# rrwick/Porechop

Measured on NVIDIA H100. Metric: reads/sec, higher is better.
Workload: dtype int16 (s16x2 DPX)

## Files before the change

porechop_b200/csrc/dp_core.cuh:

```cuda
#pragma once
#include <stdint.h>

#if defined(__CUDACC__)
#define PB_HD __host__ __device__ __forceinline__
#else
#define PB_HD inline
#endif

namespace pb {

#if !defined(__CUDA_ARCH__) && defined(PB_CHECK_RANGES)
void pb_range_violation();
#endif

constexpr int PB_BIAS = 24576;
constexpr int PB_NEG16 = -14000;
constexpr int PB_I16_LIMIT = 4000;
constexpr int PB_LINEAR_EXT = 4096;
constexpr int PB_CODE_SHIFT = 12;
constexpr int PB_MAX_SUBW = 4096;
constexpr uint8_t PB_PAD_H = 0x50;
constexpr uint8_t PB_PAD_V = 0x60;

constexpr int PB_REC = 9;
// ... 243 lines not shown
PB_HD uint32_t profile_from(uint32_t v2, uint32_t sf2, uint32_t bcode, const Scoring &sc) {
    const uint32_t e = (bcode & 7u) << 4;
    const uint32_t h2 = (e << 8) | (e << 24);
    return addmax2(xnor2(h2, v2), sc.subA2, sf2);
}
PB_HD uint32_t profile_plain(uint32_t sub2) { return (sub2 & 0x8000u) ? sub2 - 0x10000u : sub2; }
#define PB_PROF_ENCODE(x) profile_plain(x)
PB_HD uint32_t profile_word(int q, uint32_t bcode, const Scoring &sc, const uint8_t *adA, int mA, int padA, const uint8_t *adB,
                            int mB, int padB) {
    uint32_t v2, sf2;
    profile_row(q, sc, adA, mA, padA, adB, mB, padB, v2, sf2);
    return profile_from(v2, sf2, bcode, sc);
}

template <int R> struct TraceWords { static constexpr int value = (R <= 4) ? 1 : 2; };
template <int R> PB_HD int trace_word(int h, int r) { (void)r; return (R <= 4) ? 0 : h; }
template <int R> PB_HD int trace_shift(int h, int r) { return (R <= 4) ? (4 * r + 16 * h) : 4 * r; }

PB_HD int corr_flags(int x, int vs, int hs, int goEff) {
    const int sb = x - goEff;
    return (vs == sb ? 1 : 0) | (hs == sb ? 2 : 0);
}
struct FinalCol { int mask; int i0[2]; };
template <int R>
PB_HD void final_col_row(Lane<R> &L, const FinalCol &fc, int r, uint32_t x, uint32_t vs, uint32_t hs, const Scoring &sc) {
#pragma unroll
    for (int h = 0; h < 2; ++h) {
        const int i = fc.i0[h] + r;
        if (((fc.mask >> h) & 1) && i >= 1) {
            const int c = half16(x, h);
            if (c > L.fcBest[h]) {
                L.fcBest[h] = c; L.fcI[h] = i;
                L.fcCorr[h] = corr_flags(c, half16(vs, h), half16(hs, h), sc.goEff);
            }
        }
    }
}

#define PB_EXT(x) add2((x), sc.ge2)
template <int R, bool TRACE, bool KEEPV = false, bool PROF = false, bool FCOL = false>
PB_HD void lane_step(Lane<R> &L, uint32_t recvX, uint32_t recvV, uint32_t h2, const Scoring &sc, uint32_t *tw,
                     uint32_t *vr = nullptr, const uint32_t *subs = nullptr, const FinalCol *fc = nullptr) {
    uint32_t diagX = L.prevRecvX, upX = recvX, upV = recvV;
    uint32_t accLo = 0u, accHi = 0u;
#pragma unroll
    for (int r = 0; r < R; ++r) {
        const uint32_t sub = PROF ? subs[r] : addmax2(xnor2(h2, L.v2[r]), sc.subA2, L.sf2[r]);
        const uint32_t d = PROF ? diagX + sub : add2(diagX, sub);
#if !defined(__CUDA_ARCH__) && defined(PB_CHECK_RANGES)
        if (PROF && d != add2(diagX, (sub & 0x8000u) ? sub + 0x10000u : sub)) pb_range_violation();
#endif
        uint32_t hs, vs, s;
        if (TRACE) {
            const uint32_t bl = 1u << trace_shift<R>(0, r);
            const uint32_t bh = 1u << trace_shift<R>(1, r);
            const int alu_sites = (r & 1) ? (PB_FLAG_ALU_B) : (PB_FLAG_ALU_A);
            hs = max2acc((alu_sites & 1) != 0, PB_EXT(L.Hs[r]), L.X[r], accLo, bl << 3, accHi, bh << 3);
            vs = max2acc((alu_sites & 2) != 0, PB_EXT(upV), upX, accLo, bl << 2, accHi, bh << 2);
            const uint32_t gmx = max2acc((alu_sites & 4) != 0, vs, hs, accLo, bl << 1, accHi, bh << 1);
            s = max2acc((alu_sites & 8) != 0, d, gmx, accLo, bl, accHi, bh);
        } else {
            hs = addmax2(L.Hs[r], sc.ge2, L.X[r]);
            vs = addmax2(upV, sc.ge2, upX);
            s = max3(d, vs, hs);
        }
        diagX = L.X[r];
        const uint32_t xn = subm2(s, sc.goMag2);
        L.X[r] = xn; L.Hs[r] = hs;
        if (KEEPV) vr[r] = vs;
        if (FCOL) final_col_row<R>(L, *fc, r, xn, vs, hs, sc);
        upX = xn; upV = vs;
    }
    if (TRACE) {
        if (TraceWords<R>::value == 1) tw[0] = accLo + accHi; else { tw[0] = accLo; tw[1] = accHi; }
    }
    L.prevRecvX = recvX;
    L.botX = upX; L.botV = upV;
}

template <int R>
PB_HD void lane_track_lastrow(Lane<R> &L, int j, const Scoring &sc) {
    bool plo, phi;
    const uint32_t nb = max2p(L.lrBest2, L.botX, plo, phi);
    (void)sc;
    if (!(plo && phi)) {
        L.lrBest2 = nb;
        if (!plo) { L.lrJ[0] = j; L.lrV2 = (L.lrV2 & 0xFFFF0000u) | (L.botV & 0xFFFFu); L.lrH2 = (L.lrH2 & 0xFFFF0000u) | (L.Hs[R - 1] & 0xFFFFu); }
        if (!phi) { L.lrJ[1] = j; L.lrV2 = (L.lrV2 & 0xFFFFu) | (L.botV & 0xFFFF0000u); L.lrH2 = (L.lrH2 & 0xFFFFu) | (L.Hs[R - 1] & 0xFFFF0000u); }
    }
}

template <int R, bool FCOL = true>
PB_HD void lane_track_general(Lane<R> &L, int g, int j, const HalfGeom &A, const HalfGeom &B, const uint32_t *vr,
                              const Scoring &sc) {
#pragma unroll
    for (int h = 0; h < 2; ++h) {
        const HalfGeom &H = h ? B : A;
        if (j < H.n) {
            const int c = half16(L.botX, h);
            if (c > half16(L.lrBest2, h)) {
                const uint32_t keep = h ? 0xFFFFu : 0xFFFF0000u;
                L.lrBest2 = (L.lrBest2 & keep) | (L.botX & ~keep);
                L.lrV2 = (L.lrV2 & keep) | (L.botV & ~keep);
                L.lrH2 = (L.lrH2 & keep) | (L.Hs[R - 1] & ~keep);
                L.lrJ[h] = j;
            }
        } else if (FCOL && j == H.n) {
#pragma unroll
            for (int r = 0; r < R; ++r) {
                const int i = g * R + r + 1 - H.pad;
                if (i >= 1) {
                    const int c = half16(L.X[r], h);
                    if (c > L.fcBest[h]) {
                        L.fcBest[h] = c; L.fcI[h] = i;
                        L.fcCorr[h] = corr_flags(c, half16(vr[r], h), half16(L.Hs[r], h), sc.goEff);
                    }
                }
            }
        }
    }
}

struct ScoutCand { int fcBest, fcI, fcCorr, lrBest, lrJ, lrCorr; };
template <int R>
PB_HD ScoutCand make_cand(const Lane<R> &L, int h, const Scoring &sc) {
    ScoutCand c;
    c.fcBest = L.fcBest[h] < 0 ? -0x40000000 : L.fcBest[h] - PB_BIAS - sc.goEff;
    c.fcI = L.fcI[h]; c.fcCorr = L.fcCorr[h];
    c.lrBest = half16(L.lrBest2, h) - PB_BIAS - sc.goEff; c.lrJ = L.lrJ[h];
    c.lrCorr = L.lrJ[h] > 0 ? corr_flags(half16(L.lrBest2, h), half16(L.lrV2, h), half16(L.lrH2, h), sc.goEff) : 0;
    return c;
}
PB_HD EndCell scout_combine(const ScoutCand *c, int G, const HalfGeom &H) {
    EndCell e;
    if (H.n <= 0 || H.m <= 0) { e.j = 0; e.i = 0; e.score = PB_SCORE_EMPTY; e.corr = 0; return e; }
    const ScoutCand &lr = c[G - 1];
    int best = lr.lrBest, bj = lr.lrJ, bi = H.m, corr = lr.lrCorr;
    for (int g = 0; g < G; ++g) {
        if (c[g].fcBest > best) { best = c[g].fcBest; bj = H.n; bi = c[g].fcI; corr = c[g].fcCorr; }
    }
    e.j = bj; e.i = bi; e.score = best; e.corr = corr;
    return e;
}

template <class NibFn, class EqFn>
struct RandomCursor {
    NibFn nib; EqFn eqf; int j, i;
    PB_HD RandomCursor(NibFn n, EqFn e, int j0, int i0) : nib(n), eqf(e), j(j0), i(i0) {}
    PB_HD uint32_t flags() { return nib(j, i); }
    PB_HD bool eq() { return eqf(j, i); }
    PB_HD void move(bool consR, bool consA) { j -= consR ? 1 : 0; i -= consA ? 1 : 0; }
};

template <class Cursor>
PB_HD int traceback_stats_cur(Cursor &cur, const EndCell &end, bool linear, int col0, int n_total, int m, int32_t *rec) {
    if (end.score == PB_SCORE_EMPTY) {
        rec[0] = -1; rec[1] = 0; rec[2] = -1; rec[3] = 0; rec[4] = PB_SCORE_EMPTY;
        rec[5] = 0; rec[6] = 0; rec[7] = 0; rec[8] = 0;
        return 0;
    }
    int j = end.j, i = end.i;
    int L = 0, matches = 0;
    int pv = 0, ph = 0, tv = 0, th = 0;
    int dPV = 0, dPH = 0, dTV = 0, dTH = 0;
    int dir = 0;
    uint32_t b = 0;
    if (j > 0 && i > 0) {
        b = cur.flags();
        dir = (b & 1u) ? 0 : ((b & 2u) ? 1 : 2);
        if (!linear) {
            if (end.corr & 1) dir = 1; else if (end.corr & 2) dir = 2;
        }
    }
    while (j > 0 && i > 0) {
        const bool isD = dir == 0, isV = dir == 1, isH = dir == 2;
        const bool consR = !isV, consA = !isH;
        if (isD && cur.eq()) ++matches;
        const bool inPV = pv == L, inPH = ph == L;
        if (inPV) { if (isV) ++pv; else dPV = isD ? 1 : 0; }
        if (inPH) { if (isH) ++ph; else dPH = isD ? 1 : 0; }
        if (isV) ++tv; else { tv = 0; dTV = isD ? 1 : 0; }
        if (isH) ++th; else { th = 0; dTH = isD ? 1 : 0; }
        const bool ext = !linear && (isV ? ((b & 4u) && i != 1) : (isH && (b & 8u) && j != 1));
        ++L;
        if (consR) --j;
        if (consA) --i;
        cur.move(consR, consA);
        if (j > 0 && i > 0) {
            b = cur.flags();
            if (!ext) dir = (b & 1u) ? 0 : ((b & 2u) ? 1 : 2);
        }
    }
    const bool haveR = pv < L, haveA = ph < L;
    const int lastR_k = pv, lastR_i = end.i - pv, lastR_uA = dPV;
    const int lastA_k = ph, lastA_j = end.j - ph, lastA_uR = dPH;
    const int firstR_k = L - 1 - tv, firstR_i = i + tv + dTV, firstR_uA = dTV;
    const int firstA_k = L - 1 - th, firstA_j = j + th + dTH, firstA_uR = dTH;
    int status = (j == 0 && i > 0 && col0 > 0) ? 1 : 0;

    const int a = col0 + j, bb = i;
    const int jend = col0 + end.j;
    const int c = n_total - jend, e = m - end.i;
    const int Ltot = a + bb + L + c + e;
#define PB_COL(k) (a + bb + (L - 1 - (k)))
    int r0, AB_r0, a0, RB_a0;
    if (a > 0) { r0 = 0; AB_r0 = 0; }
    else if (haveR) { r0 = PB_COL(firstR_k); AB_r0 = firstR_i - firstR_uA; }
    else { r0 = bb + L; AB_r0 = end.i; }
    if (bb > 0) { a0 = 0; RB_a0 = 0; }
    else if (haveA) { a0 = PB_COL(firstA_k); RB_a0 = col0 + firstA_j - firstA_uR; }
    else { a0 = a + L + c; RB_a0 = n_total; }
    int rs, as;
    int start;
    if (r0 >= a0) { start = r0; rs = 0; as = AB_r0; } else { start = a0; as = 0; rs = RB_a0; }
    int r1, AB_r1, a1, RB_a1;
    if (c > 0) { r1 = Ltot - 1; AB_r1 = m; }
    else if (haveR) { r1 = PB_COL(lastR_k); AB_r1 = lastR_i - lastR_uA; }
    else { r1 = a - 1; AB_r1 = 0; }
    if (e > 0) { a1 = Ltot - 1; RB_a1 = n_total; }
    else if (haveA) { a1 = PB_COL(lastA_k); RB_a1 = col0 + lastA_j - lastA_uR; }
    else { a1 = a + bb - 1; RB_a1 = 0; }
#undef PB_COL
    int re, ae, endc;
    if (r1 <= a1) { endc = r1; re = n_total - 1; ae = AB_r1; } else { endc = a1; ae = m - 1; re = RB_a1; }
    rec[0] = rs; rec[1] = re; rec[2] = as; rec[3] = ae; rec[4] = end.score;
    rec[5] = matches; rec[6] = endc - start + 1; rec[7] = matches; rec[8] = a1 - a0 + 1;
    return status;
}

template <class NibFn, class EqFn>
PB_HD int traceback_stats(NibFn nib, EqFn eq, const EndCell &end, bool linear, int col0, int n_total, int m,
                          int32_t *rec) {
    RandomCursor<NibFn, EqFn> cur(nib, eq, end.j, end.i);
    return traceback_stats_cur(cur, end, linear, col0, n_total, m, rec);
}

PB_HD int32_t end_trim_candidate(const int32_t *r, int is_start, int32_t end_size, int32_t extra_trim, int32_t min_trim,
                                 const int32_t *cmin, int32_t cmin_len, int *overflow) {
    const bool failed = r[0] == -1 && r[4] == PB_SCORE_EMPTY;
    if (failed) return 0;
    const int32_t l = r[6], c = r[5];
    if (l < 0 || l >= cmin_len) { *overflow = 1; return 0; }
    if (c < cmin[l]) return 0;
    const int32_t rs = r[0], re = r[1] + 1;
    if (re - rs < min_trim) return 0;
    if (is_start) return (re == end_size) ? 0 : re + extra_trim;
    return (rs == 0) ? 0 : (end_size - rs) + extra_trim;
}
PB_HD bool middle_hit(const int32_t *r, const int32_t *cmin, int32_t cmin_len, int *overflow) {
    const int32_t l = r[8], c = r[7];
    if (l < 0 || l >= cmin_len) { *overflow = 1; return false; }
    return l > 0 && c >= cmin[l];
}
PB_HD uint32_t score_pair(const int32_t *r, int *overflow) {
    if (r[0] == -1 && r[4] == PB_SCORE_EMPTY) return 1u << 16;
    if ((uint32_t)r[7] > 0xFFFFu || (uint32_t)r[8] > 0xFFFFu) { *overflow = 1; return 0u; }
    return (uint32_t)r[7] | ((uint32_t)r[8] << 16);
}

}
```

porechop_b200/csrc/kernels.cuh:

```cuda
#pragma once
#include <cuda_runtime.h>
#include <stdint.h>
#include <string.h>
#include "dp_core.cuh"

namespace pb {

constexpr int PB_WARPS_PER_BLOCK = 4;
#ifndef PB_TRACE_MIN_BLOCKS
#define PB_TRACE_MIN_BLOCKS 6
#endif
#ifndef PB_TRACE_MIN_BLOCKS_WIDE
#define PB_TRACE_MIN_BLOCKS_WIDE 5
#endif
constexpr int PB_SCRATCH_WORDS = 32 * 2 * 6;
constexpr int PB_TCHUNK = 4;

__device__ __forceinline__ uint32_t encode_word(uint32_t w) {
    return encode_byte(w & 0xFFu) | (encode_byte((w >> 8) & 0xFFu) << 8) | (encode_byte((w >> 16) & 0xFFu) << 16) |
           (encode_byte(w >> 24) << 24);
}
__global__ void encode_kernel(const uint8_t *__restrict__ in, uint8_t *__restrict__ out, int64_t n) {
    int64_t i = ((int64_t)blockIdx.x * blockDim.x + threadIdx.x) * 16;
    const int64_t stride = (int64_t)gridDim.x * blockDim.x * 16;
    for (; i < n; i += stride) {
        if (i + 16 <= n && ((((uintptr_t)in) | ((uintptr_t)out)) & 15) == 0) {
            uint4 v = *reinterpret_cast<const uint4 *>(in + i);
            v.x = encode_word(v.x); v.y = encode_word(v.y); v.z = encode_word(v.z); v.w = encode_word(v.w);
            *reinterpret_cast<uint4 *>(out + i) = v;
        } else {
            for (int64_t k = i; k < n && k < i + 16; ++k) out[k] = (uint8_t)encode_byte(in[k]);
        }
    }
}

__global__ void unpack_kernel(const uint8_t *__restrict__ in, uint8_t *__restrict__ out, int64_t n) {
    int64_t i = ((int64_t)blockIdx.x * blockDim.x + threadIdx.x) * 16;
    const int64_t stride = (int64_t)gridDim.x * blockDim.x * 16;
    for (; i < n; i += stride) {
        if (i + 16 <= n && ((((uintptr_t)in) & 7) | (((uintptr_t)out) & 15)) == 0) {
            const uint2 p = *reinterpret_cast<const uint2 *>(in + (i >> 1));
            uint4 v;
            unpack_nibbles8(p.x, v.x, v.y);
            unpack_nibbles8(p.y, v.z, v.w);
            *reinterpret_cast<uint4 *>(out + i) = v;
        } else {
            for (int64_t k = i; k < n && k < i + 16; ++k) out[k] = (uint8_t)unpack_nibble1(in[k >> 1], (int)(k & 1));
        }
    }
}

__global__ void max_len_kernel(const int64_t *__restrict__ off, int64_t n, unsigned long long *out) {
    int64_t i = (int64_t)blockIdx.x * blockDim.x + threadIdx.x;
    unsigned long long v = 0;
    for (; i < n; i += (int64_t)gridDim.x * blockDim.x) {
        unsigned long long l = (unsigned long long)(off[i + 1] - off[i]);
        v = l > v ? l : v;
    }
    for (int o = 16; o > 0; o >>= 1) { unsigned long long w = __shfl_xor_sync(0xffffffffu, v, o); v = w > v ? w : v; }
    if ((threadIdx.x & 31) == 0 && v) atomicMax(out, v);
}

constexpr int PB_ORDER_BINS = 2048;
__device__ __forceinline__ int order_bin(int64_t len, int64_t max_len) {
    int64_t b = (len * (PB_ORDER_BINS - 1)) / (max_len > 0 ? max_len : 1);
    if (b > PB_ORDER_BINS - 1) b = PB_ORDER_BINS - 1;
    return (PB_ORDER_BINS - 1) - (int)b;
}
__global__ void order_hist_kernel(const int64_t *__restrict__ off, int64_t n, int64_t max_len, unsigned *__restrict__ bins) {
    int64_t i = (int64_t)blockIdx.x * blockDim.x + threadIdx.x;
    if (i < n) atomicAdd(&bins[order_bin(off[i + 1] - off[i], max_len)], 1u);
}
__global__ void order_scan_kernel(unsigned *bins) {
    __shared__ unsigned sh[PB_ORDER_BINS];
    for (int i = threadIdx.x; i < PB_ORDER_BINS; i += blockDim.x) sh[i] = bins[i];
    __syncthreads();
    if (threadIdx.x == 0) {
        unsigned run = 0;
        for (int i = 0; i < PB_ORDER_BINS; ++i) { unsigned v = sh[i]; sh[i] = run; run += v; }
    }
    __syncthreads();
    for (int i = threadIdx.x; i < PB_ORDER_BINS; i += blockDim.x) bins[i] = sh[i];
}
__global__ void order_scatter_kernel(const int64_t *__restrict__ off, int64_t n, int64_t max_len, unsigned *__restrict__ bins,
                                     int32_t *__restrict__ order) {
    int64_t i = (int64_t)blockIdx.x * blockDim.x + threadIdx.x;
    if (i < n) {
        unsigned pos = atomicAdd(&bins[order_bin(off[i + 1] - off[i], max_len)], 1u);
        order[pos] = (int32_t)i;
    }
}

struct TaskSrc {
    const Task *tasks;
    int64_t n_tasks;
    const int32_t *cls_ad;
    int32_t n_cls_ad;
    int32_t n_adapters;
    int64_t n_seqs;
    const int64_t *seq_off;
    const int32_t *ad_off;
    const int32_t *seq_order;
};

__device__ __forceinline__ Task cross_task(const TaskSrc &ts, int64_t k) {
    const int n_full = ts.n_cls_ad / 2;
    const int64_t paired = (int64_t)n_full * 2 * ts.n_seqs;
    int64_t s; int a;
    if (k < paired) {
        int64_t q, rem;
        if (paired <= 0xFFFFFFFFll) {
            const uint32_t d = (uint32_t)(2 * ts.n_seqs), q32 = (uint32_t)k / d;
            q = q32; rem = (uint32_t)k - q32 * d;
        } else {
            q = k / (2 * ts.n_seqs); rem = k - q * (2 * ts.n_seqs);
        }
        s = rem >> 1; a = __ldg(ts.cls_ad + 2 * q + (rem & 1));
    } else {
        s = k - paired; a = __ldg(ts.cls_ad + ts.n_cls_ad - 1);
    }
    if (ts.seq_order) s = __ldg(ts.seq_order + s);
    Task t;
    const int64_t o0 = __ldg(ts.seq_off + s), o1 = __ldg(ts.seq_off + s + 1);
    const int32_t a0 = __ldg(ts.ad_off + a), a1 = __ldg(ts.ad_off + a + 1);
    t.seq_off = o0;
    t.n = (int32_t)(o1 - o0);
    t.m = a1 - a0;
    t.ad_off = a0;
    t.out_idx = (int32_t)(s * ts.n_adapters + a);
    t.flags = 0; t.end_j = 0; t.end_i = 0; t.end_corr = 0; t.end_score = 0;
    t.col0 = 0; t.n_total = t.n; t.pad0 = t.pad1 = t.pad2 = 0;
    return t;
}
__global__ void build_tasks_pairs_kernel(Task *__restrict__ tasks, int64_t n_tasks, const int32_t *__restrict__ order,
                                         const int32_t *__restrict__ pair_seq, const int32_t *__restrict__ pair_ad,
                                         const int64_t *__restrict__ seq_off, const int32_t *__restrict__ ad_off) {
    int64_t k = (int64_t)blockIdx.x * blockDim.x + threadIdx.x;
    if (k >= n_tasks) return;
    int32_t p = order[k];
    int64_t s = pair_seq[p]; int a = pair_ad[p];
    Task t;
    t.seq_off = seq_off[s];
    t.n = (int32_t)(seq_off[s + 1] - seq_off[s]);
    t.m = ad_off[a + 1] - ad_off[a];
    t.ad_off = ad_off[a];
    t.out_idx = p;
    t.flags = 0; t.end_j = 0; t.end_i = 0; t.end_corr = 0; t.end_score = 0;
    t.col0 = 0; t.n_total = t.n; t.pad0 = t.pad1 = t.pad2 = 0;
    tasks[k] = t;
}

__device__ __forceinline__ Task get_task(const TaskSrc &ts, int64_t idx) {
    Task t;
    if (idx < ts.n_tasks) {
        if (ts.tasks == nullptr) return cross_task(ts, idx);
        const int4 *p = reinterpret_cast<const int4 *>(ts.tasks + idx);
        int4 *q = reinterpret_cast<int4 *>(&t);
        q[0] = __ldcs(p); q[1] = __ldcs(p + 1); q[2] = __ldcs(p + 2); q[3] = __ldcs(p + 3);
    } else {
        t.seq_off = 0; t.n = 0; t.m = 0; t.ad_off = 0; t.out_idx = -1; t.flags = 0; t.end_j = 0; t.end_i = 0;
        t.end_corr = 0; t.end_score = 0; t.col0 = 0; t.n_total = 0; t.pad0 = t.pad1 = t.pad2 = 0;
    }
    return t;
}

__global__ void window_tasks_kernel(const TaskSrc ts, const EndCell *__restrict__ ends, Task *__restrict__ out,
                                    int wnum, int wden, int tight, unsigned long long *__restrict__ window_cells) {
    const int64_t n_tasks = ts.n_tasks;
    int64_t k = (int64_t)blockIdx.x * blockDim.x + threadIdx.x;
    unsigned long long cells = 0;
    if (k < n_tasks) {
        Task t = get_task(ts, k);
        EndCell e = ends[k];
        if (t.n > 0 && t.m > 0) {
            const int64_t W = window_cols(t.m, e.i, e.score, wnum, wden, tight != 0);
            int64_t c0 = (int64_t)e.j - W;
            if (c0 < 0) c0 = 0;
            t.col0 = (int32_t)c0;
            t.seq_off += c0;
            t.n = e.j - (int32_t)c0;
            t.flags = TASK_END_GIVEN | (c0 > 0 ? TASK_LEFT_INF : 0);
            t.end_j = t.n; t.end_i = e.i; t.end_corr = e.corr; t.end_score = e.score;
            cells = (unsigned long long)t.n * (unsigned long long)t.m;
        } else {
            t.n = 0; t.flags = TASK_END_GIVEN; t.end_j = 0; t.end_i = 0; t.end_corr = 0; t.end_score = PB_SCORE_EMPTY;
        }
        out[k] = t;
    }
    for (int o = 16; o > 0; o >>= 1) cells += __shfl_xor_sync(0xffffffffu, cells, o);
    if ((threadIdx.x & 31) == 0 && cells && window_cells) atomicAdd(window_cells, cells);
}


__device__ __forceinline__ uint32_t pack_bases(uint32_t bA, uint32_t bB) {
    return __byte_perm(bA, bB, 0x4101);
}

constexpr int PB_STAGE_COLS = 4;
constexpr int PB_CODE_TAB_WORDS = 256 / 4;
template <int G>
__device__ __forceinline__ void stage_columns(uint32_t *hbuf, int g, const uint8_t *seqA, int nA, const uint8_t *seqB, int nB,
                                              int nmax, bool ascii, const uint8_t *code_tab) {
    for (int c0 = g; c0 < nmax; c0 += PB_STAGE_COLS * G) {
        uint32_t bA[PB_STAGE_COLS], bB[PB_STAGE_COLS];
#pragma unroll
        for (int k = 0; k < PB_STAGE_COLS; ++k) {
            const int c = c0 + k * G;
            bA[k] = (c < nA) ? (uint32_t)__ldcs(seqA + c) : (uint32_t)PB_PAD_H;
            bB[k] = (c < nB) ? (uint32_t)__ldcs(seqB + c) : (uint32_t)PB_PAD_H;
        }
        if (ascii) {
#pragma unroll
            for (int k = 0; k < PB_STAGE_COLS; ++k) {
                const int c = c0 + k * G;
                if (c < nA) bA[k] = code_tab[bA[k]];
                if (c < nB) bB[k] = code_tab[bB[k]];
            }
        }
#pragma unroll
        for (int k = 0; k < PB_STAGE_COLS; ++k) {
            const int c = c0 + k * G;
            if (c < nmax) hbuf[c] = pack_bases(bA[k], bB[k]);
        }
    }
}

template <int G, int R, bool HBUF_SMEM>
__global__ void __launch_bounds__(PB_WARPS_PER_BLOCK * 32, G <= 8 ? PB_TRACE_MIN_BLOCKS : PB_TRACE_MIN_BLOCKS_WIDE)
trace_kernel(const TaskSrc ts, const uint8_t *__restrict__ seq,
             const uint8_t *__restrict__ ads, Scoring sc, int32_t *__restrict__ out, uint32_t *__restrict__ gtrace,
             int max_steps, int max_n, int seq_ascii, int *__restrict__ status) {
    constexpr int SPW = 32 / G;
    constexpr int WPS = TraceWords<R>::value;
    extern __shared__ uint32_t smem[];
    const uint8_t *code_tab = reinterpret_cast<const uint8_t *>(smem);
    if (seq_ascii) {
        for (int w = threadIdx.x; w < PB_CODE_TAB_WORDS; w += blockDim.x)
            smem[w] = encode_byte(4u * w) | (encode_byte(4u * w + 1) << 8) | (encode_byte(4u * w + 2) << 16) |
                      (encode_byte(4u * w + 3) << 24);
        __syncthreads();
    }
    uint32_t *const warp_smem = smem + (seq_ascii ? PB_CODE_TAB_WORDS : 0);
    const int warp = threadIdx.x >> 5, lane = threadIdx.x & 31;
    const int grp = lane / G, g = lane % G;
    const int warps_per_block = blockDim.x >> 5;
    const int64_t total_warps = (int64_t)gridDim.x * warps_per_block;
    const int64_t wglobal = (int64_t)blockIdx.x * warps_per_block + warp;
    const int64_t n_tasks = ts.n_tasks;
    const int64_t n_slots = (n_tasks + 1) / 2;
    const int64_t n_wslots = (n_slots + SPW - 1) / SPW;

    const size_t trace_words = (size_t)((max_steps + PB_TCHUNK - 1) / PB_TCHUNK) * PB_TCHUNK * WPS * 32;
    const size_t gwarp_words = trace_words + (HBUF_SMEM ? 0 : (((size_t)SPW * max_n + 31) & ~(size_t)31));
    uint32_t *gw = gtrace + (size_t)wglobal * gwarp_words;
    uint32_t *tr = gw;
    const int hb_words = HBUF_SMEM ? SPW * max_n : 0;
    const int per_warp_words = hb_words + PB_SCRATCH_WORDS;
    uint32_t *wsm = warp_smem + (size_t)warp * per_warp_words;
    uint32_t *hbuf = HBUF_SMEM ? (wsm + grp * max_n) : (gw + trace_words + (size_t)grp * max_n);
    ScoutCand *cand = reinterpret_cast<ScoutCand *>(wsm + hb_words);
    for (int64_t ws = wglobal; ws < n_wslots; ws += total_warps) {
        const int64_t slot = ws * SPW + grp;
        int nA, nB, mA, mB, nmax, nmin;
        bool need_track;
        Lane<R> L;
        {
            const Task tA = get_task(ts, slot * 2);
            const Task tB = get_task(ts, slot * 2 + 1);
            nA = tA.n; nB = tB.n; mA = tA.m; mB = tB.m;
            nmax = max(nA, nB);
            stage_columns<G>(hbuf, g, seq + tA.seq_off, nA, seq + tB.seq_off, nB, nmax, seq_ascii != 0, code_tab);
            lane_init<R>(L, g, G, sc, ads + tA.ad_off, mA, (tA.flags & TASK_LEFT_INF) != 0, ads + tB.ad_off, mB,
                         (tB.flags & TASK_LEFT_INF) != 0);
            const bool emptyA = nA <= 0 || mA <= 0, emptyB = nB <= 0 || mB <= 0;
            nmin = emptyA ? nB : (emptyB ? nA : min(nA, nB));
            need_track = !((tA.flags & TASK_END_GIVEN) && (tB.flags & TASK_END_GIVEN));
        }
        int T = nmax > 0 ? nmax + G - 1 : 0;
        T = __reduce_max_sync(0xffffffffu, T);
        __syncwarp();

        const int T4 = (T + PB_TCHUNK - 1) & ~(PB_TCHUNK - 1);
        constexpr int TWARM = (G - 1 + PB_TCHUNK - 1) & ~(PB_TCHUNK - 1);
        int tfast = need_track ? (nmin - 1) : nmax;
        tfast = __reduce_min_sync(0xffffffffu, max(tfast, 0)) & ~(PB_TCHUNK - 1);
#ifdef PB_EXPERIMENT_ALL_HOT
#define PB_HOT_COL(j) max(min((j) - 1, nmax - 1), 0)
#else
#define PB_HOT_COL(j) ((j) - 1)
#endif
        for (int t0 = 0; t0 < T4; t0 += PB_TCHUNK) {
            uint4 acc[WPS];
#ifdef PB_EXPERIMENT_ALL_HOT
            if (true) {
#else
            if (t0 >= TWARM && t0 < tfast) {
#endif
                uint32_t buf[PB_TCHUNK][WPS];
#pragma unroll
                for (int u = 0; u < PB_TCHUNK; ++u) {
                    uint32_t recvS = __shfl_up_sync(0xffffffffu, L.botX, 1, G);
                    uint32_t recvV = __shfl_up_sync(0xffffffffu, L.botV, 1, G);
                    if (g == 0) { recvS = sc.borderX2; recvV = sc.negb2; }
                    const int j = t0 + u - g + 1;
                    lane_step<R, true, false>(L, recvS, recvV, hbuf[PB_HOT_COL(j)], sc, buf[u]);
                    if (need_track) lane_track_lastrow<R>(L, j, sc);
                }
#pragma unroll
                for (int w = 0; w < WPS; ++w) acc[w] = make_uint4(buf[0][w], buf[1][w], buf[2][w], buf[3][w]);
            } else {
#pragma unroll
                for (int w = 0; w < WPS; ++w) acc[w] = make_uint4(0u, 0u, 0u, 0u);
#pragma unroll 1
                for (int u = 0; u < PB_TCHUNK; ++u) {
                    const int t = t0 + u;
                    uint32_t recvS = __shfl_up_sync(0xffffffffu, L.botX, 1, G);
                    uint32_t recvV = __shfl_up_sync(0xffffffffu, L.botV, 1, G);
                    if (g == 0) { recvS = sc.borderX2; recvV = sc.negb2; }
                    const int j = t - g + 1;
                    uint32_t tw[WPS];
#pragma unroll
                    for (int w = 0; w < WPS; ++w) tw[w] = 0u;
                    const bool in = j >= 1 && j <= nmax;
                    const bool fin = in && need_track && j >= nmin;
                    const bool any_fin = !__all_sync(0xffffffffu, !fin);
                    if (in) {
                        if (any_fin) {
                            FinalCol fc;
                            fc.mask = fin ? ((j == nA ? 1 : 0) | (j == nB ? 2 : 0)) : 0;
                            fc.i0[0] = g * R + 1 - (G * R - mA); fc.i0[1] = g * R + 1 - (G * R - mB);
                            lane_step<R, true, false, false, true>(L, recvS, recvV, hbuf[j - 1], sc, tw, nullptr, nullptr, &fc);
                            if (need_track) lane_track_general<R, false>(L, g, j, make_geom(nA, mA, G, R), make_geom(nB, mB, G, R), nullptr, sc);
                        } else {
                            lane_step<R, true, false>(L, recvS, recvV, hbuf[j - 1], sc, tw);
                            if (need_track) lane_track_lastrow<R>(L, j, sc);
                        }
                    }
#pragma unroll
                    for (int w = 0; w < WPS; ++w) {
                        if (u == 0) acc[w].x = tw[w]; else if (u == 1) acc[w].y = tw[w]; else if (u == 2) acc[w].z = tw[w]; else acc[w].w = tw[w];
                    }
                }
            }
#pragma unroll
            for (int w = 0; w < WPS; ++w)
                *reinterpret_cast<uint4 *>(tr + (((size_t)(t0 / PB_TCHUNK) * WPS + w) * 32 + lane) * PB_TCHUNK) = acc[w];
        }
        cand[lane] = make_cand<R>(L, 0, sc);
        cand[32 + lane] = make_cand<R>(L, 1, sc);
        __syncwarp();
#ifndef PB_EXPERIMENT_SKIP_TRACEBACK
        if (g < 2) {
            const int h = g;
            const Task tk = get_task(ts, slot * 2 + h);
            const HalfGeom gh = make_geom(tk.n, tk.m, G, R);
            if (tk.out_idx >= 0) {
                EndCell end;
                if (tk.flags & TASK_END_GIVEN) {
                    end.j = tk.end_j; end.i = tk.end_i; end.score = tk.end_score; end.corr = tk.end_corr;
                    if (tk.n_total <= 0 || tk.m <= 0) end.score = PB_SCORE_EMPTY;
                } else {
                    end = scout_combine(cand + h * 32 + grp * G, G, gh);
                }
#ifdef PB_EXPERIMENT_ALL_HOT
                end.j = min(end.j, tk.n); end.i = min(end.i, tk.m);
#endif
                struct Cursor {
                    const uint32_t *base;
                    const uint32_t *hp;
                    const uint8_t *ap;
                    int gg, r, t, key, h;
                    uint4 cv;
                    __device__ __forceinline__ uint32_t flags() {
                        const int k = (t >> 2) * (WPS * 32) + gg;
                        if (k != key) { cv = *reinterpret_cast<const uint4 *>(base + (size_t)k * PB_TCHUNK); key = k; }
                        const uint32_t lo = (t & 1) ? cv.y : cv.x, hi = (t & 1) ? cv.w : cv.z;
                        return (((t & 2) ? hi : lo) >> trace_shift<R>(h, r)) & 15u;
                    }
                    __device__ __forceinline__ bool eq() { return ((*hp >> (8 + 16 * h)) & 0xFFu) == (uint32_t)__ldg(ap); }
                    __device__ __forceinline__ void move(bool consR, bool consA) {
                        if (consA) { --ap; if (r == 0) { r = R - 1; --gg; --t; } else --r; }
                        if (consR) { --t; --hp; }
                    }
                } cur;
                {
                    const int q = max(end.i + gh.pad - 1, 0);
                    cur.gg = q / R; cur.r = q % R; cur.t = end.j - 1 + cur.gg; cur.key = -1; cur.h = h;
                    cur.base = tr + ((size_t)trace_word<R>(h, 0) * 32 + grp * G) * PB_TCHUNK;
                    cur.hp = hbuf + end.j - 1; cur.ap = ads + tk.ad_off + end.i - 1;
                    cur.cv = make_uint4(0u, 0u, 0u, 0u);
                }
                int32_t rec[PB_REC];
                int st = traceback_stats_cur(cur, end, sc.linear != 0, tk.col0, tk.n_total, tk.m, rec);
                if (st) atomicOr(status, 1);
                int32_t *o = out + (size_t)tk.out_idx * PB_REC;
#pragma unroll
                for (int k = 0; k < PB_REC; ++k) __stcs(o + k, rec[k]);
            }
        }
#endif
        __syncwarp();
        for (int l = lane; l < T4 * WPS; l += 32)
            asm volatile("discard.global.L2 [%0], 128;" ::"l"(tr + (size_t)l * 32) : "memory");
        __syncwarp();
    }
}

constexpr int PB_RING = 64;
constexpr int PB_BLK = 32;
#ifndef PB_RING32
typedef uint16_t ring_t;
__device__ __forceinline__ ring_t ring_pack(uint32_t bA, uint32_t bB) { return (ring_t)(bA | (bB << 8)); }
__device__ __forceinline__ uint32_t ring_bases(uint32_t x) { return __byte_perm(x, 0u, 0x1404); }
#else
typedef uint32_t ring_t;
__device__ __forceinline__ ring_t ring_pack(uint32_t bA, uint32_t bB) { return pack_bases(bA, bB); }
__device__ __forceinline__ uint32_t ring_bases(uint32_t x) { return x; }
#endif

template <int CPL>
__device__ __forceinline__ uint64_t load_cols(const uint8_t *p) {
    if (CPL == 8) {
        const uintptr_t a = reinterpret_cast<uintptr_t>(p);
        const unsigned long long *q = reinterpret_cast<const unsigned long long *>(a & ~(uintptr_t)7);
        const unsigned sh = (unsigned)(a & 7) * 8;
        const unsigned long long lo = __ldcs(q), hi = __ldcs(q + 1);
        return sh ? ((lo >> sh) | (hi << (64 - sh))) : lo;
    } else if (CPL == 4) {
        const uintptr_t a = reinterpret_cast<uintptr_t>(p);
        const unsigned *q = reinterpret_cast<const unsigned *>(a & ~(uintptr_t)3);
        const unsigned sh = (unsigned)(a & 3) * 8;
        const unsigned lo = __ldcs(q), hi = __ldcs(q + 1);
        return (uint64_t)__funnelshift_r(lo, hi, sh);
    } else {
        uint64_t v = 0;
#pragma unroll
        for (int c = 0; c < CPL; ++c) v |= (uint64_t)__ldcs(p + c) << (8 * c);
        return v;
    }
}

#ifndef PB_SCORE_MIN_BLOCKS
#define PB_SCORE_MIN_BLOCKS 6
#endif
#ifndef PB_SCORE_MIN_BLOCKS_NOPROF
#define PB_SCORE_MIN_BLOCKS_NOPROF 5
#endif
template <int G, int R> struct ProfGeom {
    static constexpr int ROWS = G * R;
    static constexpr int PLANE = 4 * G;
    static constexpr int STRIDE = 6 * ROWS + 16;
    static constexpr int RING = PB_RING + 2 * G;
};
template <int G, int R, bool PROF = false>
__global__ void __launch_bounds__(PB_WARPS_PER_BLOCK * 32, PROF ? PB_SCORE_MIN_BLOCKS : PB_SCORE_MIN_BLOCKS_NOPROF)
score_kernel(const TaskSrc ts, unsigned long long *__restrict__ counter,
             const uint8_t *__restrict__ seq, const uint8_t *__restrict__ ads, Scoring sc, EndCell *__restrict__ ends) {
    constexpr int SPW = 32 / G;
    constexpr int CPL = PB_BLK / G;
    static_assert(!PROF || R == 8, "the profile variant fetches 8 operands per step");
    __shared__ ScoutCand scratch[PB_WARPS_PER_BLOCK][2 * 32];
    __shared__ __align__(16) ring_t rings[PB_WARPS_PER_BLOCK][SPW][ProfGeom<G, R>::RING];
    __shared__ __align__(16) uint32_t profs[PROF ? PB_WARPS_PER_BLOCK * SPW * ProfGeom<G, R>::STRIDE : 4];
    const int warp = threadIdx.x >> 5, lane = threadIdx.x & 31;
    const int grp = lane / G, g = lane % G;
    const unsigned gmask = (G == 32) ? 0xffffffffu : (((1u << G) - 1u) << (grp * G));
    const int64_t n_tasks = ts.n_tasks;
    const int64_t n_slots = (n_tasks + 1) / 2;
    ScoutCand *cand = scratch[warp];
    ring_t *ring = rings[warp][grp];
    uint32_t *myprof = profs + (PROF ? ((size_t)(warp * SPW + grp) * ProfGeom<G, R>::STRIDE + g * 4) : 0);

    Lane<R> L;
    HalfGeom gA, gB;
    const uint8_t *seqA = seq, *seqB = seq;
    int64_t slot = -1;
    int nA = 0, nB = 0, nmax = 0, nmin = 0, T = 0, t = 0;
    bool exhausted = false;
    uint64_t pendA = 0, pendB = 0;
    gA = make_geom(0, 0, G, R); gB = gA;
    L.botX = sc.borderX2; L.botV = sc.negb2;
    uint32_t top_keep = g != 0 ? 1u : 0u;
    const uint32_t top_addS = g == 0 ? sc.borderX2 : 0u, top_addV = g == 0 ? sc.negb2 : 0u;
    asm volatile("" : "+r"(top_keep));
    if (PROF) {
        for (int c = g; c < PB_RING; c += G) ring[c] = (ring_t)0;
        __syncwarp();
    }

    auto fetch = [&](int blk) {
        const int c0 = blk * PB_BLK + g * CPL;
        pendA = (c0 < nA) ? load_cols<CPL>(seqA + c0) : 0ull;
        if (!PROF) pendB = (c0 < nB) ? load_cols<CPL>(seqB + c0) : 0ull;
    };
    auto store = [&](int blk) {
        const int c0 = blk * PB_BLK + g * CPL;
        uint32_t e[CPL];
        if (PROF && c0 + CPL <= nA) {
#pragma unroll
            for (int c = 0; c < CPL; ++c) e[c] = (uint32_t)((pendA >> (8 * c + 4)) & 0xFu) * (uint32_t)ProfGeom<G, R>::ROWS;
        } else {
#pragma unroll
            for (int c = 0; c < CPL; ++c) {
                const int col = c0 + c;
                const uint32_t bA = (col < nA) ? (uint32_t)((pendA >> (8 * c)) & 0xFFu) : (uint32_t)PB_PAD_H;
                const uint32_t bB = PROF ? bA : ((col < nB) ? (uint32_t)((pendB >> (8 * c)) & 0xFFu) : (uint32_t)PB_PAD_H);
                e[c] = PROF ? (bA >> 4) * (uint32_t)ProfGeom<G, R>::ROWS : (uint32_t)ring_pack(bA, bB);
            }
        }
        ring_t *dst = ring + (c0 & (PB_RING - 1));
#ifndef PB_RING32
        if (CPL == 8) *reinterpret_cast<uint4 *>(dst) = make_uint4(e[0] | (e[1 % CPL] << 16), e[2 % CPL] | (e[3 % CPL] << 16),
                                                                    e[4 % CPL] | (e[5 % CPL] << 16), e[6 % CPL] | (e[7 % CPL] << 16));
        else if (CPL == 4) *reinterpret_cast<uint2 *>(dst) = make_uint2(e[0] | (e[1 % CPL] << 16), e[2 % CPL] | (e[3 % CPL] << 16));
        else if (CPL == 2) *reinterpret_cast<uint32_t *>(dst) = e[0] | (e[1 % CPL] << 16);
        else dst[0] = (ring_t)e[0];
#else
#pragma unroll
        for (int c = 0; c < CPL; ++c) dst[c] = (ring_t)e[c];
#endif
    };

    for (;;) {
        __syncwarp();
        if (!exhausted) {
            if (t >= T) {
                if (slot >= 0) {
                    cand[lane] = make_cand<R>(L, 0, sc);
                    cand[32 + lane] = make_cand<R>(L, 1, sc);
                    __syncwarp(gmask);
                    if (g < 2) {
                        const int64_t ti = slot * 2 + g;
                        if (ti < n_tasks) ends[ti] = scout_combine(cand + g * 32 + grp * G, G, g ? gB : gA);
                    }
                    __syncwarp(gmask);
                }
                unsigned long long s = 0;
                if (g == 0) s = atomicAdd(counter, 1ull);
                s = __shfl_sync(gmask, s, 0, G);
                if ((int64_t)s >= n_slots) {
                    exhausted = true; slot = -1; T = 0; t = 0; nmax = 0; nmin = 0; nA = nB = 0;
                } else {
                    slot = (int64_t)s;
                    const Task tA = get_task(ts, slot * 2);
                    const Task tB = get_task(ts, slot * 2 + 1);
                    nA = tA.n; nB = tB.n;
                    gA = make_geom(tA.n, tA.m, G, R); gB = make_geom(tB.n, tB.m, G, R);
                    nmax = max(nA, nB);
                    seqA = seq + tA.seq_off; seqB = seq + tB.seq_off;
                    lane_init<R>(L, g, G, sc, ads + tA.ad_off, tA.m, false, ads + tB.ad_off, tB.m, false);
                    if (PROF) {
#pragma unroll
// ... 401 lines not shown
```

Measured before the change: 213.5 million.

## Derive traceback match count from score and streamline trace cursor stepping

The traceback now skips the per-diagonal-step base comparison and computes the match count algebraically from the end score, diagonal count, gap count and gap-open count whenever match and mismatch scores differ. The first/last-boundary bookkeeping is rebuilt around tracking the positions directly. A new TraceCursor walks the packed trace words with an incremental shift and chunk index and reloads only when it crosses a chunk. Task metadata is staged into shared memory so the traceback stage does not re-read it from global memory. This cuts global loads and ALU work on the serial traceback path, but relies on the score identity being exact, including gap-open accounting at the path end.

```diff
diff --git a/porechop_b200/csrc/dp_core.cuh b/porechop_b200/csrc/dp_core.cuh
--- a/porechop_b200/csrc/dp_core.cuh
+++ b/porechop_b200/csrc/dp_core.cuh
@@ -419,50 +419,54 @@
     PB_HD void move(bool consR, bool consA) { j -= consR ? 1 : 0; i -= consA ? 1 : 0; }
 };
 
-template <class Cursor>
-PB_HD int traceback_stats_cur(Cursor &cur, const EndCell &end, bool linear, int col0, int n_total, int m, int32_t *rec) {
+template <bool FROM_SCORE = false, class Cursor>
+PB_HD int traceback_stats_cur(Cursor &cur, const EndCell &end, bool linear, int col0, int n_total, int m, int32_t *rec,
+                              const Scoring *sc = nullptr) {
     if (end.score == PB_SCORE_EMPTY) {
         rec[0] = -1; rec[1] = 0; rec[2] = -1; rec[3] = 0; rec[4] = PB_SCORE_EMPTY;
         rec[5] = 0; rec[6] = 0; rec[7] = 0; rec[8] = 0;
         return 0;
     }
     int j = end.j, i = end.i;
-    int L = 0, matches = 0;
-    int pv = 0, ph = 0, tv = 0, th = 0;
-    int dPV = 0, dPH = 0, dTV = 0, dTH = 0;
-    int dir = 0;
+    int L = 0, matches = 0, opens = 0;
+    int kR1 = 0, iR1 = 0, kA1 = 0, jA1 = 0;
+    int kR2 = 0, iR2 = 0, kA2 = 0, jA2 = 0;
+    int consR = 1, consA = 1;
     uint32_t b = 0;
+    bool ext = false;
     if (j > 0 && i > 0) {
         b = cur.flags();
-        dir = (b & 1u) ? 0 : ((b & 2u) ? 1 : 2);
+        consR = (b & 3u) != 2u; consA = (b & 3u) != 0u;
         if (!linear) {
-            if (end.corr & 1) dir = 1; else if (end.corr & 2) dir = 2;
+            if (end.corr & 1) { consR = 0; consA = 1; } else if (end.corr & 2) { consR = 1; consA = 0; }
         }
     }
     while (j > 0 && i > 0) {
-        const bool isD = dir == 0, isV = dir == 1, isH = dir == 2;
-        const bool consR = !isV, consA = !isH;
-        if (isD && cur.eq()) ++matches;
-        const bool inPV = pv == L, inPH = ph == L;
-        if (inPV) { if (isV) ++pv; else dPV = isD ? 1 : 0; }
-        if (inPH) { if (isH) ++ph; else dPH = isD ? 1 : 0; }
-        if (isV) ++tv; else { tv = 0; dTV = isD ? 1 : 0; }
-        if (isH) ++th; else { th = 0; dTH = isD ? 1 : 0; }
-        const bool ext = !linear && (isV ? ((b & 4u) && i != 1) : (isH && (b & 8u) && j != 1));
-        ++L;
+        const bool isD = (consR & consA) != 0;
+        if (!FROM_SCORE && isD && cur.eq()) ++matches;
+        ext = (b & (linear ? 0u : (!consR ? 4u : (!consA ? 8u : 0u)))) != 0u;
+        if (FROM_SCORE && !isD && !ext) ++opens;
+        const bool onR = j == end.j, onA = i == end.i;
         if (consR) --j;
         if (consA) --i;
-        cur.move(consR, consA);
+        if (onR) { kR1 = L; iR1 = i; }
+        if (onA) { kA1 = L; jA1 = j; }
+        if (consR) { kR2 = L; iR2 = i; }
+        if (consA) { kA2 = L; jA2 = j; }
+        ++L;
+        cur.move(consR != 0, consA != 0);
         if (j > 0 && i > 0) {
             b = cur.flags();
-            if (!ext) dir = (b & 1u) ? 0 : ((b & 2u) ? 1 : 2);
+            if (!ext) { consR = (b & 3u) != 2u; consA = (b & 3u) != 0u; }
         }
     }
-    const bool haveR = pv < L, haveA = ph < L;
-    const int lastR_k = pv, lastR_i = end.i - pv, lastR_uA = dPV;
-    const int lastA_k = ph, lastA_j = end.j - ph, lastA_uR = dPH;
-    const int firstR_k = L - 1 - tv, firstR_i = i + tv + dTV, firstR_uA = dTV;
-    const int firstA_k = L - 1 - th, firstA_j = j + th + dTH, firstA_uR = dTH;
+    if (FROM_SCORE) {
+        if (ext) ++opens;
+        const int diag = (end.i - i) + (end.j - j) - L, gaps = L - diag;
+        const int gapcost = linear ? sc->ge * gaps : sc->go * opens + sc->ge * (gaps - opens);
+        matches = (end.score - sc->mi * diag - gapcost) / (sc->ma - sc->mi);
+    }
+    const bool haveR = j < end.j, haveA = i < end.i;
     int status = (j == 0 && i > 0 && col0 > 0) ? 1 : 0;
 
     const int a = col0 + j, bb = i;
@@ -472,20 +476,20 @@
 #define PB_COL(k) (a + bb + (L - 1 - (k)))
     int r0, AB_r0, a0, RB_a0;
     if (a > 0) { r0 = 0; AB_r0 = 0; }
-    else if (haveR) { r0 = PB_COL(firstR_k); AB_r0 = firstR_i - firstR_uA; }
+    else if (haveR) { r0 = PB_COL(kR2); AB_r0 = iR2; }
     else { r0 = bb + L; AB_r0 = end.i; }
     if (bb > 0) { a0 = 0; RB_a0 = 0; }
-    else if (haveA) { a0 = PB_COL(firstA_k); RB_a0 = col0 + firstA_j - firstA_uR; }
+    else if (haveA) { a0 = PB_COL(kA2); RB_a0 = col0 + jA2; }
     else { a0 = a + L + c; RB_a0 = n_total; }
     int rs, as;
     int start;
     if (r0 >= a0) { start = r0; rs = 0; as = AB_r0; } else { start = a0; as = 0; rs = RB_a0; }
     int r1, AB_r1, a1, RB_a1;
     if (c > 0) { r1 = Ltot - 1; AB_r1 = m; }
-    else if (haveR) { r1 = PB_COL(lastR_k); AB_r1 = lastR_i - lastR_uA; }
+    else if (haveR) { r1 = PB_COL(kR1); AB_r1 = iR1; }
     else { r1 = a - 1; AB_r1 = 0; }
     if (e > 0) { a1 = Ltot - 1; RB_a1 = n_total; }
-    else if (haveA) { a1 = PB_COL(lastA_k); RB_a1 = col0 + lastA_j - lastA_uR; }
+    else if (haveA) { a1 = PB_COL(kA1); RB_a1 = col0 + jA1; }
     else { a1 = a + bb - 1; RB_a1 = 0; }
 #undef PB_COL
     int re, ae, endc;
diff --git a/porechop_b200/csrc/kernels.cuh b/porechop_b200/csrc/kernels.cuh
--- a/porechop_b200/csrc/kernels.cuh
+++ b/porechop_b200/csrc/kernels.cuh
@@ -13,7 +13,8 @@
 #ifndef PB_TRACE_MIN_BLOCKS_WIDE
 #define PB_TRACE_MIN_BLOCKS_WIDE 5
 #endif
-constexpr int PB_SCRATCH_WORDS = 32 * 2 * 6;
+constexpr int PB_TB_WORDS = 16 * 12;
+constexpr int PB_SCRATCH_WORDS = 32 * 2 * 6 + PB_TB_WORDS;
 constexpr int PB_TCHUNK = 4;
 
 __device__ __forceinline__ uint32_t encode_word(uint32_t w) {
@@ -225,6 +226,63 @@
     }
 }
 
+struct TbTask {
+    int32_t out_idx, flags, col0, n_total, ad_off, end_j, end_i, end_score, n, m, pad0, pad1;
+};
+static_assert(sizeof(TbTask) * 16 == PB_TB_WORDS * 4, "PB_TB_WORDS holds 16 TbTasks");
+
+template <int R, int WPS>
+struct TraceCursor {
+    const uint4 *base;
+    const uint32_t *hp;
+    const uint8_t *ap;
+    uint4 cv;
+    int k;
+    int u, s, h;
+    int fresh;
+#ifdef PB_EXPERIMENT_PATH_STEPS
+    int steps;
+#endif
+    __device__ __forceinline__ void init(const uint32_t *tr_half, int end_j, int end_i, int pad, int hh, const uint32_t *hbuf,
+                                         const uint8_t *ad) {
+        const int q = max(end_i + pad - 1, 0), gg = q / R, r = q % R, t = end_j - 1 + gg;
+        h = hh;
+        base = reinterpret_cast<const uint4 *>(tr_half);
+        k = (t >> 2) * (WPS * 32) + gg;
+        u = t & 3; s = 28 - trace_shift<R>(h, r); fresh = 1;
+        hp = hbuf + end_j - 1; ap = ad + end_i - 1;
+        cv = make_uint4(0u, 0u, 0u, 0u);
+#ifdef PB_EXPERIMENT_PATH_STEPS
+        steps = 0;
+#endif
+    }
+    __device__ __forceinline__ uint32_t flags() {
+        if (fresh) { cv = base[k]; fresh = 0; }
+        const uint32_t lo = (u & 1) ? cv.y : cv.x, hi = (u & 1) ? cv.w : cv.z;
+        return (((u & 2) ? hi : lo) << s) >> 28;
+    }
+    __device__ __forceinline__ bool eq() { return ((*hp >> (8 + 16 * h)) & 0xFFu) == (uint32_t)__ldg(ap); }
+    __device__ __forceinline__ void move(bool consR, bool consA) {
+        const int s0 = 28 - trace_shift<R>(h, 0);
+        const bool wrap = consA && s == s0;
+        s = wrap ? s0 - 4 * (R - 1) : (consA ? s + 4 : s);
+        const int dt = (consR ? 1 : 0) + (wrap ? 1 : 0);
+        const bool back = u < dt;
+        u = (u - dt) & 3;
+        k -= (back ? WPS * 32 : 0) + (wrap ? 1 : 0);
+        fresh |= (back || wrap) ? 1 : 0;
+        if (consA) --ap;
+        if (consR) --hp;
+#ifdef PB_EXPERIMENT_PATH_STEPS
+        ++steps;
+#endif
+    }
+};
+
+#ifdef PB_EXPERIMENT_PATH_STEPS
+extern "C" { __device__ unsigned long long pb_path_stats[4]; }
+#endif
+
 template <int G, int R, bool HBUF_SMEM>
 __global__ void __launch_bounds__(PB_WARPS_PER_BLOCK * 32, G <= 8 ? PB_TRACE_MIN_BLOCKS : PB_TRACE_MIN_BLOCKS_WIDE)
 trace_kernel(const TaskSrc ts, const uint8_t *__restrict__ seq,
@@ -259,6 +317,7 @@
     uint32_t *wsm = warp_smem + (size_t)warp * per_warp_words;
     uint32_t *hbuf = HBUF_SMEM ? (wsm + grp * max_n) : (gw + trace_words + (size_t)grp * max_n);
     ScoutCand *cand = reinterpret_cast<ScoutCand *>(wsm + hb_words);
+    TbTask *tbt = reinterpret_cast<TbTask *>(cand + 64) + grp * 2;
     for (int64_t ws = wglobal; ws < n_wslots; ws += total_warps) {
         const int64_t slot = ws * SPW + grp;
         int nA, nB, mA, mB, nmax, nmin;
@@ -268,6 +327,14 @@
             const Task tA = get_task(ts, slot * 2);
             const Task tB = get_task(ts, slot * 2 + 1);
             nA = tA.n; nB = tB.n; mA = tA.m; mB = tB.m;
+            if (g < 2) {
+                const Task &tk = g ? tB : tA;
+                TbTask b;
+                b.out_idx = tk.out_idx; b.flags = tk.flags | (tk.end_corr << 8); b.col0 = tk.col0; b.n_total = tk.n_total;
+                b.ad_off = tk.ad_off; b.end_j = tk.end_j; b.end_i = tk.end_i; b.end_score = tk.end_score;
+                b.n = tk.n; b.m = tk.m; b.pad0 = b.pad1 = 0;
+                tbt[g] = b;
+            }
             nmax = max(nA, nB);
             stage_columns<G>(hbuf, g, seq + tA.seq_off, nA, seq + tB.seq_off, nB, nmax, seq_ascii != 0, code_tab);
             lane_init<R>(L, g, G, sc, ads + tA.ad_off, mA, (tA.flags & TASK_LEFT_INF) != 0, ads + tB.ad_off, mB,
@@ -350,54 +417,45 @@
         cand[32 + lane] = make_cand<R>(L, 1, sc);
         __syncwarp();
 #ifndef PB_EXPERIMENT_SKIP_TRACEBACK
+#ifdef PB_EXPERIMENT_PATH_STEPS
+        int path_steps = 0;
+#endif
         if (g < 2) {
             const int h = g;
-            const Task tk = get_task(ts, slot * 2 + h);
+            const TbTask tk = tbt[h];
             const HalfGeom gh = make_geom(tk.n, tk.m, G, R);
             if (tk.out_idx >= 0) {
                 EndCell end;
                 if (tk.flags & TASK_END_GIVEN) {
-                    end.j = tk.end_j; end.i = tk.end_i; end.score = tk.end_score; end.corr = tk.end_corr;
-                    if (tk.n_total <= 0 || tk.m <= 0) end.score = PB_SCORE_EMPTY;
+                    end.j = tk.end_j; end.i = tk.end_i; end.score = tk.end_score; end.corr = tk.flags >> 8;
+                    if (tk.n_total <= 0 || gh.m <= 0) end.score = PB_SCORE_EMPTY;
                 } else {
                     end = scout_combine(cand + h * 32 + grp * G, G, gh);
                 }
 #ifdef PB_EXPERIMENT_ALL_HOT
-                end.j = min(end.j, tk.n); end.i = min(end.i, tk.m);
-#endif
-                struct Cursor {
-                    const uint32_t *base;
-                    const uint32_t *hp;
-                    const uint8_t *ap;
-                    int gg, r, t, key, h;
-                    uint4 cv;
-                    __device__ __forceinline__ uint32_t flags() {
-                        const int k = (t >> 2) * (WPS * 32) + gg;
-                        if (k != key) { cv = *reinterpret_cast<const uint4 *>(base + (size_t)k * PB_TCHUNK); key = k; }
-                        const uint32_t lo = (t & 1) ? cv.y : cv.x, hi = (t & 1) ? cv.w : cv.z;
-                        return (((t & 2) ? hi : lo) >> trace_shift<R>(h, r)) & 15u;
-                    }
-                    __device__ __forceinline__ bool eq() { return ((*hp >> (8 + 16 * h)) & 0xFFu) == (uint32_t)__ldg(ap); }
-                    __device__ __forceinline__ void move(bool consR, bool consA) {
-                        if (consA) { --ap; if (r == 0) { r = R - 1; --gg; --t; } else --r; }
-                        if (consR) { --t; --hp; }
-                    }
-                } cur;
-                {
-                    const int q = max(end.i + gh.pad - 1, 0);
-                    cur.gg = q / R; cur.r = q % R; cur.t = end.j - 1 + cur.gg; cur.key = -1; cur.h = h;
-                    cur.base = tr + ((size_t)trace_word<R>(h, 0) * 32 + grp * G) * PB_TCHUNK;
-                    cur.hp = hbuf + end.j - 1; cur.ap = ads + tk.ad_off + end.i - 1;
-                    cur.cv = make_uint4(0u, 0u, 0u, 0u);
-                }
+                end.j = min(end.j, gh.n); end.i = min(end.i, gh.m);
+#endif
+                TraceCursor<R, WPS> cur;
+                cur.init(tr + ((size_t)trace_word<R>(h, 0) * 32 + grp * G) * PB_TCHUNK, end.j, end.i, gh.pad, h, hbuf,
+                         ads + tk.ad_off);
                 int32_t rec[PB_REC];
-                int st = traceback_stats_cur(cur, end, sc.linear != 0, tk.col0, tk.n_total, tk.m, rec);
+                const int st = sc.ma != sc.mi ? traceback_stats_cur<true>(cur, end, sc.linear != 0, tk.col0, tk.n_total, gh.m, rec, &sc)
+                                              : traceback_stats_cur(cur, end, sc.linear != 0, tk.col0, tk.n_total, gh.m, rec);
                 if (st) atomicOr(status, 1);
                 int32_t *o = out + (size_t)tk.out_idx * PB_REC;
 #pragma unroll
                 for (int k = 0; k < PB_REC; ++k) __stcs(o + k, rec[k]);
-            }
-        }
+#ifdef PB_EXPERIMENT_PATH_STEPS
+                path_steps = cur.steps;
+                atomicAdd(&pb_path_stats[0], (unsigned long long)cur.steps);
+                atomicAdd(&pb_path_stats[1], 1ull);
+#endif
+            }
+        }
+#ifdef PB_EXPERIMENT_PATH_STEPS
+        path_steps = __reduce_max_sync(0xffffffffu, path_steps);
+        if (lane == 0) { atomicAdd(&pb_path_stats[2], (unsigned long long)path_steps); atomicAdd(&pb_path_stats[3], 1ull); }
+#endif
 #endif
         __syncwarp();
         for (int l = lane; l < T4 * WPS; l += 32)
```

Measured after the change: 224.1 million, median of 6. 4.9% higher.
